# VinAIResearch/Point-Unet

Hardware: AMD Instinct MI355X
Metric: points_per_sec_forward (higher is better)
Workload: dtype f32

## Files before the change

### point-unet_amd/csrc/attpool.h

```cpp
#pragma once

#include "common.h"
#include "rowgemm.h"

namespace ps {

struct Att32Weights {
    const float* w1 = nullptr;
    const float* w2 = nullptr;
    const float* wb1 = nullptr;
    const float* wb2 = nullptr;
    const float* w1b = nullptr;
    const float* w2b = nullptr;
    const float* wb1b = nullptr;
    const float* wb2b = nullptr;
};
void pack_b3(const float* W, int cin, int cout, uint16_t* out);
void pack_b3_locse(const float* W1, int cout, uint16_t* out);
void pack_p32(const float* W, int cin, int cout, float* out);
void pack_p32_locse(const float* W1, int cout, float* out);

struct AttStage {
    const float* xyz = nullptr;
    const int32_t* idx = nullptr;
    const int32_t* order = nullptr;
    const float* fg = nullptr;
    const PackedLinear* lfa1 = nullptr;
    const PackedLinear* lfa2 = nullptr;
    const PackedLinear* wbot = nullptr;
    const PackedLinear* wfull = nullptr;
    int ldf = 0;
    float* agg = nullptr;
    int64_t n_total = 0, n_cloud = 0;
    int d = 0, k = 16;
    const Att32Weights* p32 = nullptr;
    const float* lane = nullptr;
};

constexpr int kLaneB1 = 0, kLaneW1 = 8, kLaneB2 = 88, kLaneW2 = 96, kLaneWfc = 160, kLaneImageFloats = 416;
void pack_lane_image(const float* W1, const float* b1, const float* W2, const float* b2, const float* wfc_scaled, float* out);

bool att_pool32_fits(const AttStage& s);
int att_pool32_stage(ps_context* c, const AttStage& s);
bool att_pool32b_fits(const AttStage& s);
int att_pool32b_stage(ps_context* c, const AttStage& s);

bool att_lane_fits(const ps_context* c, const AttStage& s);
int att_lane_stage(ps_context* c, const AttStage& s);
int att_lane_pass_points();

int att_pool_stage(ps_context* c, const AttStage& s);
int att_pool_form(const ps_context* c, const AttStage& s);
int att_pool16_stage(ps_context* c, const AttStage& s);

}
```

### point-unet_amd/csrc/attpool.hip

```cpp
#include "attpool.h"
#include "mfma_tile.h"

namespace ps {

struct AttArgs {
    const float* xyz;
    const int32_t* idx;
    const int32_t* order;
    const float* fg;
    const float* w1p; const float* b1;
    const float* w2p; const float* b2;
    const float* wbp;
    const float* wfp;
    float* agg;
    int n_total, n_cloud, ldf;
};

struct PointWalk {
    int t, end, stride;
    __device__ __forceinline__ PointWalk(int n_total, int units_per_wg, int unit_in_wg)
    {
        const int per_xcd = (n_total + 7) >> 3;
        const int xcd = blockIdx.x & 7, slot = blockIdx.x >> 3, slots = gridDim.x >> 3;
        t = xcd * per_xcd + slot * units_per_wg + unit_in_wg;
// ... 454 lines not shown
        if (smem > 48 * 1024) PS_HIP(hipFuncSetAttribute(reinterpret_cast<const void*>(kern), hipFuncAttributeMaxDynamicSharedMemorySize, (int)smem));
        const int blocks = (std::min(a.n_total, 256 * 16) + 7) & ~7;
        hipLaunchKernelGGL(kern, dim3(blocks), dim3(WAVES * 64), smem, c->stream, a);
        PS_HIP(hipGetLastError());
        return PS_OK;
    }
    constexpr int WAVES = per_wave * 4 <= 160 * 1024 ? 4 : (per_wave * 2 <= 160 * 1024 ? 2 : 1);
    static_assert(per_wave * WAVES <= 160 * 1024, "attention tile does not fit the LDS");
    const size_t smem = per_wave * WAVES;
    auto kern = att_kernel<D, STAGE, KN, WAVES, false>;
    if (smem > 48 * 1024) PS_HIP(hipFuncSetAttribute(reinterpret_cast<const void*>(kern), hipFuncAttributeMaxDynamicSharedMemorySize, (int)smem));
    const int blocks = (std::min(ceil_div(a.n_total, WAVES), 256 * 8) + 7) & ~7;
    hipLaunchKernelGGL(kern, dim3(blocks), dim3(WAVES * 64), smem, c->stream, a);
    PS_HIP(hipGetLastError());
    return PS_OK;
}

template <int STAGE, int KN>
static int dispatch_d(ps_context* c, int d, const AttArgs& a)
{
    switch (d) {
        case 16: return launch_att<16, STAGE, KN>(c, a);
        case 32: return launch_att<32, STAGE, KN>(c, a);
        case 64: return launch_att<64, STAGE, KN>(c, a);
        case 128: return launch_att<128, STAGE, KN>(c, a);
        case 256: return launch_att<256, STAGE, KN>(c, a);
        case 512: return launch_att<512, STAGE, KN>(c, a);
        default: set_error("att_pool: d_out %d is not a compiled size (16,32,64,128,256,512)", d); return PS_EINVAL;
    }
}

int att_pool_stage(ps_context* c, const AttStage& s)
{
    if (c->att_bf16x3 && att_pool32b_fits(s)) return att_pool32b_stage(c, s);
    if (att_pool32_fits(s)) return att_pool32_stage(c, s);
    if (att_lane_fits(c, s)) return att_lane_stage(c, s);
    return att_pool16_stage(c, s);
}

int att_pool_form(const ps_context* c, const AttStage& s)
{
    if (c->att_bf16x3 && att_pool32b_fits(s)) return 1;
    if (att_pool32_fits(s)) return 2;
    return att_lane_fits(c, s) ? 4 : 3;
}

int att_pool16_stage(ps_context* c, const AttStage& s)
{
    AttArgs a;
    a.xyz = s.xyz; a.idx = s.idx; a.order = s.order; a.fg = s.fg;
    a.w1p = s.lfa1->wp; a.b1 = s.lfa1->bias;
    a.w2p = s.lfa2 ? s.lfa2->wp : nullptr; a.b2 = s.lfa2 ? s.lfa2->bias : nullptr;
    a.wbp = s.wbot ? s.wbot->wp : nullptr;
    a.wfp = s.wfull ? s.wfull->wp : nullptr;
    a.agg = s.agg;
    a.n_total = (int)s.n_total; a.n_cloud = (int)s.n_cloud;
    a.ldf = s.ldf;
    if (s.n_total <= 0) return PS_OK;
    const int stage = s.lfa2 ? 2 : 1;
    if (s.wfull) {
        PS_CHECK((uint64_t)s.n_total * (uint64_t)std::max(s.d, std::max(s.ldf, 3 * 1)) < (1ull << 32) && (uint64_t)s.n_total * s.k < (1ull << 32),
                 "att_pool: level too large for 32-bit element offsets");
        if (s.k == 16) return stage == 1 ? dispatch_direct<1, 16>(c, s.d, a) : dispatch_direct<2, 16>(c, s.d, a);
        if (s.k == 32) return stage == 1 ? dispatch_direct<1, 32>(c, s.d, a) : dispatch_direct<2, 32>(c, s.d, a);
        set_error("att_pool: k_n %d is not a compiled size (16, 32)", s.k);
        return PS_EINVAL;
// ... 9 lines not shown
```

### point-unet_amd/csrc/attpool_lane.hip

```cpp
#include "attpool.h"
#include "mfma_tile.h"

namespace ps {

void pack_lane_image(const float* W1, const float* b1, const float* W2, const float* b2, const float* wfc_scaled, float* out)
{
    std::memcpy(out + kLaneB1, b1, sizeof(float) * 8);
    std::memcpy(out + kLaneW1, W1, sizeof(float) * 80);
    if (b2) std::memcpy(out + kLaneB2, b2, sizeof(float) * 8);
    else std::memset(out + kLaneB2, 0, sizeof(float) * 8);
    if (W2) std::memcpy(out + kLaneW2, W2, sizeof(float) * 64);
    else std::memset(out + kLaneW2, 0, sizeof(float) * 64);
    std::memcpy(out + kLaneWfc, wfc_scaled, sizeof(float) * 256);
}

namespace {

struct AttLaneArgs {
    const float* xyz;
    const int32_t* idx;
    const int32_t* order;
    const float* f;
    const float* w;
    float* agg;
    int n_total, n_cloud, ldf;
};

constexpr int kLaneWaves = 4;
constexpr int kLanePts = 4;
constexpr int kLaneMaxBlocks = 256 * 8;
constexpr int kLanePitch = 17;

static_assert(kLaneB1 == 0 && kLaneW1 == 8 && kLaneB2 == 88 && kLaneW2 == 96 && kLaneWfc == 160 && kLaneImageFloats == 13 * 32, "att_lane_kernel: image layout");

using cfloat = const float __attribute__((address_space(4)));
using cfloat2 = const f32x2 __attribute__((address_space(4)));

__device__ __forceinline__ f32x2 fma2(float x, f32x2 w, f32x2 acc) { return __builtin_elementwise_fma(f32x2{x, x}, w, acc); }
__device__ __forceinline__ f32x2 leaky2(f32x2 v) { return f32x2{leaky02(v.x), leaky02(v.y)}; }

template <int STAGE>
__global__ __launch_bounds__(kLaneWaves * 64) void att_lane_kernel(AttLaneArgs a)
{
    __shared__ float smem[kLaneWaves * 64 * kLanePitch];
    const int wave = __builtin_amdgcn_readfirstlane(threadIdx.x >> 6), lane = threadIdx.x & 63;
    const int pi = lane >> 4, k = lane & 15;
    float* T = smem + wave * (64 * kLanePitch);
    float* t_row = T + lane * kLanePitch;
    const float* t_col = T + (pi * 16) * kLanePitch + k;
    cfloat* wimg = (cfloat*)(uintptr_t)a.w;

    const bool one_cloud = a.n_total == a.n_cloud;
    const int per_xcd = ((((a.n_total + 7) >> 3) + kLanePts - 1) / kLanePts) * kLanePts;
    const int w_end = min(a.n_total, (int)((blockIdx.x & 7) + 1) * per_xcd), w_slots = gridDim.x >> 3;
    for (int t = (int)(blockIdx.x & 7) * per_xcd + ((int)(blockIdx.x >> 3) * kLaneWaves + wave) * kLanePts; t < w_end; t += w_slots * kLaneWaves * kLanePts) {
        const int ti = min(t + pi, w_end - 1);
        unsigned p, base;
        if (one_cloud) {
            p = a.order ? (unsigned)a.order[ti] : (unsigned)ti;
            base = 0u;
        } else {
            base = ((unsigned)ti / (unsigned)a.n_cloud) * (unsigned)a.n_cloud;
            p = a.order ? base + (unsigned)a.order[ti] : (unsigned)ti;
        }
        const float* cp = a.xyz + 3u * p;
        const float cx = cp[0], cy = cp[1], cz = cp[2];
        const unsigned nb = base + (unsigned)a.idx[p * 16u + (unsigned)k];
        const float* np = a.xyz + 3u * nb;
        const float nx = np[0], ny = np[1], nz = np[2];
        const float4* fr = reinterpret_cast<const float4*>(a.f + nb * (unsigned)a.ldf);
        const float4 fa = fr[0], fb = fr[1];
        const float rx = cx - nx, ry = cy - ny, rz = cz - nz;
        const float dis = __builtin_amdgcn_sqrtf(rx * rx + ry * ry + rz * rz);
        const float enc[10] = {dis, rx, ry, rz, cx, cy, cz, nx, ny, nz};

        f32x2 w[2][16];
        auto fetch = [&](int c, f32x2 (&dst)[16], auto& after) {
            cfloat* wp = wimg;
            asm volatile("" : "+s"(wp), "+v"(after));
            cfloat2* w2 = reinterpret_cast<cfloat2*>(wp) + c * 16;
#pragma unroll
            for (int j = 0; j < 16; ++j) dst[j] = w2[j];
        };
        auto mac4 = [](float xv, const f32x2* wr, f32x2 (&acc)[4]) {
#pragma unroll
            for (int j = 0; j < 4; ++j) acc[j] = fma2(xv, wr[j], acc[j]);
        };
        int tie = ti;
        fetch(0, w[0], tie);
        fetch(1, w[1], tie);
        f32x2 fx[4], g2[4];
#pragma unroll
        for (int j = 0; j < 4; ++j) fx[j] = w[0][j];
#pragma unroll
        for (int q = 0; q < 3; ++q) mac4(enc[q], &w[0][4 + 4 * q], fx);
        fetch(2, w[0], fx[0]);
#pragma unroll
        for (int q = 3; q < 7; ++q) mac4(enc[q], &w[1][4 * (q - 3)], fx);
        fetch(STAGE == 2 ? 3 : 5, w[1], fx[0]);
#pragma unroll
        for (int q = 7; q < 10; ++q) mac4(enc[q], &w[0][4 * (q - 7)], fx);
#pragma unroll
        for (int j = 0; j < 4; ++j) {
            g2[j] = w[0][12 + j];
            fx[j] = leaky2(fx[j]);
        }
        if constexpr (STAGE == 2) {
            fetch(4, w[0], g2[0]);
#pragma unroll
            for (int q = 0; q < 4; ++q) mac4(q & 1 ? fx[q >> 1].y : fx[q >> 1].x, &w[1][4 * q], g2);
            fetch(5, w[1], g2[0]);
#pragma unroll
            for (int q = 4; q < 8; ++q) mac4(q & 1 ? fx[q >> 1].y : fx[q >> 1].x, &w[0][4 * (q - 4)], g2);
#pragma unroll
            for (int j = 0; j < 4; ++j) fx[j] = leaky2(g2[j]);
        }
        const float x[16] = {fa.x, fa.y, fa.z, fa.w, fb.x, fb.y, fb.z, fb.w, fx[0].x, fx[0].y, fx[1].x, fx[1].y, fx[2].x, fx[2].y, fx[3].x, fx[3].y};
        f32x2 s[8];
#pragma unroll
        for (int j = 0; j < 8; ++j) s[j] = f32x2{0.f, 0.f};
#pragma unroll
        for (int i = 0; i < 8; ++i) {
            if (i < 7) fetch(6 + i, w[i & 1], s[0]);
            const f32x2* wr = w[(i + 1) & 1];
#pragma unroll
            for (int j = 0; j < 8; ++j) s[j] = fma2(x[2 * i], wr[j], s[j]);
#pragma unroll
            for (int j = 0; j < 8; ++j) s[j] = fma2(x[2 * i + 1], wr[8 + j], s[j]);
        }
#pragma unroll
        for (int j = 0; j < 8; ++j) {
            t_row[2 * j] = s[j].x;
            t_row[2 * j + 1] = s[j].y;
        }
        wave_lds_sync();
        float sc[16];
#pragma unroll
        for (int r = 0; r < 16; ++r) sc[r] = t_col[r * kLanePitch];
        wave_lds_sync();
#pragma unroll
        for (int q = 0; q < 16; ++q) t_row[q] = x[q];
        wave_lds_sync();
        float v[16];
#pragma unroll
        for (int r = 0; r < 16; ++r) v[r] = t_col[r * kLanePitch];
        wave_lds_sync();
        float m = sc[0];
#pragma unroll
        for (int r = 1; r < 16; ++r) m = fmaxf(m, sc[r]);
        float ss[4], num[4];
#pragma unroll
        for (int g = 0; g < 4; ++g) {
            ss[g] = 0.f;
            num[g] = 0.f;
#pragma unroll
            for (int r = 4 * g; r < 4 * g + 4; ++r) {
                const float e = __builtin_amdgcn_exp2f(sc[r] - m);
                ss[g] += e;
                num[g] = __builtin_fmaf(e, v[r], num[g]);
            }
        }
        const float ssum = (ss[0] + ss[1]) + (ss[2] + ss[3]);
        const float nsum = (num[0] + num[1]) + (num[2] + num[3]);
        if (t + pi < w_end) a.agg[p * 16u + (unsigned)k] = nsum * __builtin_amdgcn_rcpf(ssum);
    }
}

}

int att_lane_pass_points() { return kLaneMaxBlocks * kLaneWaves * kLanePts; }

bool att_lane_fits(const ps_context* c, const AttStage& s)
{
    return c->att_lane && s.wfull && s.lane && s.d == 16 && s.k == 16 && s.ldf >= 8 && s.ldf % 4 == 0 &&
           (uint64_t)s.n_total * (uint64_t)std::max(s.d, std::max(s.ldf, 3)) < (1ull << 32);
}

int att_lane_stage(ps_context* c, const AttStage& s)
{
    if (!(s.wfull && s.lane && s.d == 16 && s.k == 16)) {
        set_error("att_pool(lane): d_out %d, k_n %d -- the lane kernel is compiled for d_out 16, k_n 16 and the direct formulation only", s.d, s.k);
        return PS_EINVAL;
    }
    PS_CHECK((uint64_t)s.n_total * (uint64_t)std::max(s.d, std::max(s.ldf, 3)) < (1ull << 32), "att_pool(lane): level too large for 32-bit element offsets");
    PS_CHECK(s.ldf % 4 == 0 && s.ldf >= 8, "att_pool(lane): feature rows need a stride of whole float4s");
    if (s.n_total <= 0) return PS_OK;
    AttLaneArgs a;
    a.xyz = s.xyz; a.idx = s.idx; a.order = s.order; a.f = s.fg; a.w = s.lane; a.agg = s.agg;
    a.n_total = (int)s.n_total; a.n_cloud = (int)s.n_cloud; a.ldf = s.ldf;
    const int blocks = (std::min(ceil_div(a.n_total, kLaneWaves * kLanePts), kLaneMaxBlocks) + 7) & ~7;
    if (s.lfa2) hipLaunchKernelGGL(att_lane_kernel<2>, dim3(blocks), dim3(kLaneWaves * 64), 0, c->stream, a);
    else hipLaunchKernelGGL(att_lane_kernel<1>, dim3(blocks), dim3(kLaneWaves * 64), 0, c->stream, a);
    PS_HIP(hipGetLastError());
    return PS_OK;
}

}
```

### point-unet_amd/csrc/common.h

```cpp
#pragma once

#include <hip/hip_runtime.h>

#include <cstdarg>
#include <cstdint>
#include <cstdio>
#include <cstring>
#include <map>
#include <string>
#include <vector>

#include "../../include/pointseg.h"
#include "../../include/pointseg_train_ops.h"

namespace ps {

void set_error(const char* fmt, ...);

#define PS_HIP(expr)                                                                                  \
    do {                                                                                              \
        hipError_t _e = (expr);                                                                       \
        if (_e != hipSuccess) {                                                                       \
            ps::set_error("%s failed: %s (%s:%d)", #expr, hipGetErrorString(_e), __FILE__, __LINE__); \
            return PS_EHIP;                                                                           \
// ... 92 lines not shown
    bool gather_reduce_ordered = true;
    int maxpool_bwd_ordered = 1;
    bool train_act_bf16 = true;
    int train_att_gemm_split = -1;
    bool train_att_gemm = true;
    bool train_att128_fwd_gemm = true;
    bool train_fuse_residual = true;
    bool train_merge_syncbn = true;
    int convbn_max_c = 64;
    int convbn_rect_max = 1 << 30;
    bool wgrad_debug = false;
};
void tuning_from_env(Tuning& t);
}

struct ps_context {
    int device = 0;
    ps::Tuning tune;
    hipStream_t own_stream = nullptr;
    hipStream_t stream = nullptr;
    ps::Arena knn_arena;
    ps::Arena net_arena;
    ps::Arena sample_arena;
    ps::DevBuf stage_in;
    ps::DevBuf stage_out;
    ps::DevBuf red_ws;
    ps::DevBuf wgrad_ws;
    ps::PackCache* pack_cache = nullptr;
    ps::DevBuf ops_ring[4];
    int ops_ring_pos = 0;
    bool att_bf16x3 = true;
    bool regchain_b3 = true;
    bool att_lane = true;
    bool train_b3 = true;
    bool conv_w_transposed = false;
    bool att_df_accum = false;
    const int32_t* walk_order = nullptr;
    int64_t walk_order_n = 0;
    bool pool_bwd_overwrite = false;
    bool train_bf16 = false;
    bool train_act_bf16 = false;
    bool mid_lds_attr = false;
    size_t chain_lds_attr = 48 * 1024;
    std::map<const void*, size_t> regchain_lds_attr;
    bool deferred = false;
    int32_t* h_flags = nullptr;
    unsigned pending_mask = 0;
    uint64_t builds = 0;
    uint64_t samples = 0;
    uint64_t volume_samples = 0;
    uint64_t flag_serial[8] = {};
    int flag_kind[8] = {};
    int flag_slot = 0;
    int sticky_rc = 0;
    std::string sticky_msg;
    hipEvent_t flag_ev[8] = {};
    std::vector<char> host_ring[8];
    int ring_pos = 0;
    std::vector<char>& ring_next() { ring_pos = (ring_pos + 1) & 7; return host_ring[ring_pos]; }
    int check_deferred();
    int check_flag_slot(int s);
    int defer_status(const void* d_words, size_t bytes, int kind, uint64_t serial);
    struct PinSlot { void* p = nullptr; size_t cap = 0; hipEvent_t ev = nullptr; bool busy = false; };
    PinSlot pin[16];
    int pin_pos = 0;
    int upload_async(void* dst, const void* src, size_t bytes);
// ... 69 lines not shown
```

### point-unet_amd/csrc/debug_hooks.h

```cpp
#ifndef POINTSEG_DEBUG_H
#define POINTSEG_DEBUG_H
#include "../../include/pointseg.h"
#ifdef __cplusplus
extern "C" {
#endif
int ps_debug_knn_host(const float* support, const float* queries, int64_t B, int64_t n_support,
                      int64_t n_queries, int64_t K, int32_t* out_idx);
int ps_debug_kdtree_host(const float* support, int64_t n, int32_t* vind, int32_t* nodes, float* pts,
                         int32_t* root_depth, float* bbox);
int ps_debug_kdtree_device(ps_context* ctx, const float* support, int64_t n, int32_t* vind, int32_t* nodes,
                           float* pts, int32_t* root_depth, float* bbox);
#define PS_DEBUG_KDTREE_STATS 22
int ps_debug_kdtree_device_set(ps_context* ctx, const float* support, const int32_t* n, int64_t T, const int32_t* want_copy, int32_t* vind,
                               int32_t* nodes, float* pts, int32_t* fat, int32_t* root_depth, float* bbox, float* copy, int32_t* stats);
int ps_debug_pack_weights(const float* W, int cin, int cout, int ntb, float* out);
int ps_debug_pack_b3(const float* W, int cin, int cout, uint16_t* out);
int ps_debug_pack_b3_device(ps_context* ctx, const float* W, int cin, int cout, void* out);
int ps_debug_gemm32(ps_context* ctx, int split_bf16, const float* x1, int ld1, int c1, const int32_t* g1, const float* x2, int ld2, int c2,
                    const int32_t* g2, int gm, int gn, const float* W, const float* bias, int64_t R, int cout, int leaky, float* y, int ldy);
int ps_debug_gemm32_plan(ps_context* ctx, int split_bf16, int64_t R, int cin, int cout, int* out4);

typedef struct ps_debug_chain_layer {
    const float* W;
    const float* bias;
    int cin, cout, leaky;
    float* y;
    int ldy;
    const float* extra;
    int ld_extra, c_extra;
    const int32_t* extra_gather;
} ps_debug_chain_layer;
typedef struct ps_debug_chain_desc {
    int n_layers;
    ps_debug_chain_layer layer[4];
    const float* x1; const int32_t* g1; int ld1, c1, g1m, g1n;
    const float* x2; const int32_t* g2; int ld2, c2, g2m, g2n;
    int64_t R;
} ps_debug_chain_desc;
int ps_debug_chain(ps_context* ctx, const ps_debug_chain_desc* d, int form);
int ps_debug_chain_plan(const ps_debug_chain_desc* d, int* out4);
int ps_debug_set_regchain_b3(ps_context* ctx, int on);
int ps_debug_set_att_lane(ps_context* ctx, int on);
int ps_debug_att_stage(ps_randla* net, int level, int stage, int form, const float* xyz, const int32_t* idx, const int32_t* order, const float* fg,
                       int64_t n_total, int64_t n_cloud, float* agg);
int ps_debug_att_form(ps_randla* net, int level, int stage, int k, int64_t n_total);
int ps_debug_att_lane_pass_points(void);

int ps_debug_set_tuning(ps_context* ctx, const char* field, double value);
int ps_debug_get_tuning(ps_context* ctx, const char* field, double* value);
int ps_debug_tuning_fields(char* buf, int cap);
int ps_debug_volume_sample_args_size(void);

int64_t ps_debug_scan_words(int64_t n);
int64_t ps_debug_sort_words(int64_t n);
int ps_debug_scan_launches(int64_t n);
int ps_debug_sort_launches(int64_t n, int bits);
int ps_debug_scan_u32(ps_context* ctx, const uint32_t* in, uint32_t* out, int64_t n, uint32_t* work);
int ps_debug_sort_pairs(ps_context* ctx, int key_bytes, void* k0, void* k1, uint32_t* v0, uint32_t* v1, int64_t n, int bits, uint32_t* work,
                        int* which_out);
int ps_debug_reduce_partials(ps_context* ctx, int form, const void* part, int n_part, int nv, int n0, void* out0, void* out1);

#ifdef __cplusplus
}
#endif
#endif
```

### point-unet_amd/csrc/debug_hooks.hip

```cpp
#include "common.h"

#include <cstring>
#include <vector>
#include "kdtree_build.h"
#include "kdtree_host.h"
#include "rowgemm.h"
#include "attpool.h"
#include "debug_hooks.h"
#include "randla_net.h"
#include "reduce_partials.h"
#include "sortscan.h"

using namespace ps;

extern "C" int ps_debug_volume_sample_args_size(void) { return (int)sizeof(ps_volume_sample_args); }

extern "C" int ps_debug_pack_weights(const float* W, int cin, int cout, int ntb, float* out)
{
    PS_CHECK(W && out && (ntb == 1 || ntb == 2 || ntb == 4), "ps_debug_pack_weights: bad argument");
    pack_weights(W, cin, cout, ntb, out);
    return PS_OK;
}

extern "C" int ps_debug_pack_b3(const float* W, int cin, int cout, uint16_t* out)
// ... 243 lines not shown
    s.lane = stage == 1 ? e.lane1 : e.lane2;
    int rc = PS_EINVAL;
    if (form == 4) rc = att_lane_stage(c, s);
    else if (form == 0) rc = att_pool_stage(c, s);
    else if (form == 1 && att_pool32b_fits(s)) rc = att_pool32b_stage(c, s);
    else if (form == 2 && att_pool32_fits(s)) rc = att_pool32_stage(c, s);
    else if (form == 3) rc = att_pool16_stage(c, s);
    else set_error("ps_debug_att_stage: the level (d = %d, %lld rows) does not fit the 32x32 form %d", d, (long long)n_total, form);
    (void)hipStreamSynchronize(c->stream);
    return rc;
}

extern "C" int ps_debug_att_form(ps_randla* net, int level, int stage, int k, int64_t n_total)
{
    if (!net || !net->have_weights || level < 0 || level >= net->cfg.num_layers || (stage != 1 && stage != 2) || k < 1 || n_total < 0) {
        set_error("ps_debug_att_form: bad argument");
        return -1;
    }
    const EncLevel& e = net->enc[level];
    const int d = e.d, h = d / 2;
    const bool use_g = d >= 64;
    AttStage s;
    s.lfa1 = &e.lfa1; s.lfa2 = stage == 2 ? &e.lfa2 : nullptr;
    s.wbot = use_g ? (stage == 1 ? &e.bot1 : &e.bot2) : nullptr;
    s.wfull = use_g ? nullptr : (stage == 1 ? &e.full1 : &e.full2);
    s.lane = stage == 1 ? e.lane1 : e.lane2;
    s.p32 = e.has_p32 ? &e.p32 : nullptr;
    s.n_total = n_total; s.n_cloud = n_total; s.d = d; s.k = k; s.ldf = use_g ? h + d : h;
    return att_pool_form(net->ctx, s);
}

extern "C" int ps_debug_att_lane_pass_points(void) { return att_lane_pass_points(); }

static bool is_bool(double v) { return v == 0 || v == 1; }
static bool is_int_in(double v, double lo, double hi) { return v >= lo && v <= hi && v == (double)(int64_t)v; }

#define PS_TUNING_FIELDS(X)                                                \
    X(gemm32b_min_flops, v >= 0 && v <= 1e300)                             \
    X(gemm32b_rw, v == 0 || v == 1 || v == 2)                              \
    X(gemm32b_cw, v == 0 || v == 1 || v == 2)                              \
    X(gemm32_no_sk8, is_bool(v))                                           \
    X(att64_gemm, is_bool(v))                                              \
    X(att64_occ, v == 0 || v == 1 || v == 2)                               \
    X(att_no_split, is_bool(v))                                            \
    X(wgrad_b3_min_rows, is_int_in(v, 0, (double)(1ll << 40)))             \
    X(gemm_b3_min_rows, is_int_in(v, 0, (double)(1ll << 40)))              \
    X(wgrad_wgs, is_int_in(v, 64, 4096))                                   \
    X(bn_slice, is_bool(v))                                                \
    X(inv_bucket, is_bool(v))                                              \
    X(inv_tile, v == 4096 || v == 6144 || v == 8192)                       \
    X(gather_reduce_ordered, is_bool(v))                                   \
    X(maxpool_bwd_ordered, is_bool(v))                                     \
    X(train_act_bf16, is_bool(v))                                          \
    X(train_att_gemm_split, v == -1 || v == 0 || v == 1)                   \
    X(train_att_gemm, is_bool(v))                                          \
    X(train_att128_fwd_gemm, is_bool(v))                                   \
    X(train_fuse_residual, is_bool(v))                                     \
    X(train_merge_syncbn, is_bool(v))                                      \
    X(convbn_max_c, is_int_in(v, 0, 4096))                                 \
    X(convbn_rect_max, is_int_in(v, 0, (double)(1 << 30)))                 \
    X(wgrad_debug, is_bool(v))

extern "C" int ps_debug_set_tuning(ps_context* c, const char* field, double v)
{
    PS_CHECK(c && field, "ps_debug_set_tuning: NULL argument");
#define PS_SET(f, ok)                                                                                 \
// ... 207 lines not shown
```

### point-unet_amd/csrc/randla.hip

```cpp
#include "attpool.h"
#include "common.h"
#include "randla_net.h"
#include "rowgemm.h"

#include <memory>

namespace ps {

template <int KN>
__global__ __launch_bounds__(256) void pool_max_kernel(const float* __restrict__ feat, const int32_t* __restrict__ idx, const int32_t* __restrict__ order,
                                                       float* __restrict__ out, int rows_out, int m_cloud, int n_cloud, int K, int c4 ,
                                                       unsigned char* __restrict__ ties )
{
    const int per_xcd = (rows_out + 7) >> 3;
    const int xcd = blockIdx.x & 7;
    const size_t lim = (size_t)min(rows_out, (xcd + 1) * per_xcd) * c4;
    for (size_t t = (size_t)xcd * per_xcd * c4 + (size_t)(blockIdx.x >> 3) * 256 + threadIdx.x; t < lim; t += (size_t)(gridDim.x >> 3) * 256) {
        const int r = (int)(t / c4), q = (int)(t - (size_t)r * c4);
        const int row = order ? (r / m_cloud) * m_cloud + order[r] : r;
        const int base = (row / m_cloud) * n_cloud;
        const int32_t* ix = idx + (size_t)row * K;
        const float4* f4 = reinterpret_cast<const float4*>(feat);
        float4 m;
        if constexpr (KN > 0) {
// ... 213 lines not shown
                for (size_t t = 0; t < count; ++t) tmp[t] = (float)((double)src[t] * 1.4426950408889634);
                return tmp.data();
            };
            pack_p32(scaled(W(si + 2) + (size_t)h * d, (size_t)h * d), h, d, emit_raw(&e.p32.wb1, (size_t)h * d));
            pack_p32(W(si + 4), h, h, emit_raw(&e.p32.w2, (size_t)h * h));
            pack_p32(scaled(W(si + 5) + (size_t)h * d, (size_t)h * d), h, d, emit_raw(&e.p32.wb2, (size_t)h * d));
            if (d == 64 || d == 128 || d == 256 || d == 512) {
                pack_b3_locse(W(si + 1), h, reinterpret_cast<uint16_t*>(emit_raw(&e.p32.w1b, (size_t)(h / 32) * 3 * 64 * 4)));
                pack_b3(scaled(W(si + 2) + (size_t)h * d, (size_t)h * d), h, d, reinterpret_cast<uint16_t*>(emit_raw(&e.p32.wb1b, (size_t)h * d * 3 / 2)));
                pack_b3(W(si + 4), h, h, reinterpret_cast<uint16_t*>(emit_raw(&e.p32.w2b, (size_t)h * h * 3 / 2)));
                pack_b3(scaled(W(si + 5) + (size_t)h * d, (size_t)h * d), h, d, reinterpret_cast<uint16_t*>(emit_raw(&e.p32.wb2b, (size_t)h * d * 3 / 2)));
            }
        }
        emit(e.mlp1, W(si), Bv(si), d_in, h, 1); ++si;
        emit(e.lfa1, W(si), Bv(si), 10, h, 1); ++si;
        emit(e.top1, W(si), nullptr, h, d, 0);
        emit(e.bot1, W(si) + (size_t)h * d, nullptr, h, d, 0);
        {
            std::vector<float> sc((size_t)d * d);
            for (size_t t = 0; t < sc.size(); ++t) sc[t] = (float)((double)W(si)[t] * 1.4426950408889634);
            emit(e.full1, sc.data(), nullptr, d, d, 0);
        }
        ++si;
        emit(e.att1mlp, W(si), Bv(si), d, h, 1); ++si;
        emit(e.lfa2, W(si), Bv(si), h, h, 1); ++si;
        emit(e.top2, W(si), nullptr, h, d, 0);
        emit(e.bot2, W(si) + (size_t)h * d, nullptr, h, d, 0);
        {
            std::vector<float> sc((size_t)d * d);
            for (size_t t = 0; t < sc.size(); ++t) sc[t] = (float)((double)W(si)[t] * 1.4426950408889634);
            emit(e.full2, sc.data(), nullptr, d, d, 0);
        }
        ++si;
        e.lane1 = e.lane2 = nullptr;
        if (d == 16) {
            auto scaled16 = [&](const float* src) {
                tmp.resize(256);
                for (size_t t = 0; t < 256; ++t) tmp[t] = (float)((double)src[t] * 1.4426950408889634);
                return tmp.data();
            };
            const size_t lfa1_i = si - 5, fc1_i = si - 4, lfa2_i = si - 2, fc2_i = si - 1;
            pack_lane_image(W(lfa1_i), Bv(lfa1_i), nullptr, nullptr, scaled16(W(fc1_i)), emit_raw(&e.lane1, kLaneImageFloats));
            pack_lane_image(W(lfa1_i), Bv(lfa1_i), W(lfa2_i), Bv(lfa2_i), scaled16(W(fc2_i)), emit_raw(&e.lane2, kLaneImageFloats));
        }
        emit(e.att2mlp, W(si), Bv(si), d, d, 1); ++si;
        tmp.assign((size_t)(d + d_in) * 2 * d + 2 * d, 0.f);
        std::memcpy(tmp.data(), W(si), sizeof(float) * (size_t)d * 2 * d);
        std::memcpy(tmp.data() + (size_t)d * 2 * d, W(si + 1), sizeof(float) * (size_t)d_in * 2 * d);
        float* bsum = tmp.data() + (size_t)(d + d_in) * 2 * d;
        for (int k = 0; k < 2 * d; ++k) bsum[k] = Bv(si)[k] + Bv(si + 1)[k];
        emit(e.mlp2sc, tmp.data(), bsum, d + d_in, 2 * d, 1);
        si += 2;
        d_in = 2 * d;
    }
    emit(net->decoder0, W(si), Bv(si), d_in, d_in, 1); ++si;
    net->dec.assign(cfg.num_layers, PackedLinear());
    for (int j = 0; j < cfg.num_layers; ++j) {
        emit(net->dec[j], W(si), Bv(si), net->specs[si].cin, net->specs[si].cout, 1);
        ++si;
    }
    emit(net->fc1, W(si), Bv(si), net->specs[si].cin, 64, 1); ++si;
    emit(net->fc2, W(si), Bv(si), 64, 32, 1); ++si;
    emit(net->fc, W(si), Bv(si), 32, cfg.num_classes, 0); ++si;

    PS_TRY(net->wbuf.reserve(host.size() * sizeof(float)));
    PS_HIP(hipMemcpyAsync(net->wbuf.p, host.data(), host.size() * sizeof(float), hipMemcpyHostToDevice, c->stream));
    PS_HIP(hipStreamSynchronize(c->stream));
    for (auto& p : pend) {
        p.L->wp = net->wbuf.as<float>() + p.wp_off;
        p.L->bias = net->wbuf.as<float>() + p.b_off;
        p.L->wq = p.wq_off ? net->wbuf.as<float>() + p.wq_off : nullptr;
        p.L->w32 = p.w32_off ? net->wbuf.as<float>() + p.w32_off : nullptr;
        p.L->w32b = p.w32b_off ? net->wbuf.as<float>() + p.w32b_off : nullptr;
    }
    for (auto& p : pend_raw) *p.dst = net->wbuf.as<float>() + p.off;
    net->have_weights = true;
    return PS_OK;
}

extern "C" int ps_randla_forward(ps_randla* net, const ps_pyramid* pyr, const float* features, float* logits)
{
    PS_CHECK(net && pyr && features && logits, "ps_randla_forward: NULL argument");
    if (!net->have_weights) {
        set_error("ps_randla_forward: weights not set");
// ... 66 lines not shown
    int d_in = 8;
    for (int i = 0; i < L; ++i) {
        const EncLevel& e = net->enc[i];
        const int d = e.d, h = d / 2;
        const int64_t R = B * n[i];
        const bool use_g = d >= 64;
        const int ldf = use_g ? h + d : h;
        char nm[48];
        AttStage s;
        s.xyz = pyr->xyz[i]; s.idx = pyr->neigh_idx[i]; s.order = pyr->order[i]; s.fg = fg; s.lfa1 = &e.lfa1; s.agg = agg;
        s.n_total = R; s.n_cloud = n[i]; s.d = d; s.k = cfg.k_n; s.ldf = ldf;
        s.p32 = e.has_p32 ? &e.p32 : nullptr;
        s.lane = e.lane1;
        auto feature_rows = [&](const PackedLinear& mlp, const PackedLinear& top, const RowSrc& in) -> int {
            ChainStep ch[2] = {step(mlp, fg, ldf), step(top, fg + h, ldf)};
            const int nsteps = use_g ? 2 : 1;
            if (nsteps == 2 && rowchain_fits(ch, 2, in, none)) return rowchain(c, ch, 2, in, none, R, &net->chains);
            if (nsteps == 1 && regchain_fits(ch, 1, in, none)) return rowchain(c, ch, 1, in, none, R, &net->chains);
            PS_TRY(rowgemm(c, mlp, in, none, R, fg, ldf));
            if (use_g) PS_TRY(rowgemm(c, top, src(fg, ldf, h), none, R, fg + h, ldf));
            return PS_OK;
        };
        if (i == 0 && mlp1_0_done) {
            if (use_g) {
                std::snprintf(nm, sizeof nm, "enc%d_dense", i);
                Stage st(c, nm, 1);
                PS_TRY(rowgemm(c, e.top1, src(fg, ldf, h), none, R, fg + h, ldf));
            }
        } else {
            std::snprintf(nm, sizeof nm, "enc%d_dense", i);
            Stage st(c, nm, 1);
            PS_TRY(feature_rows(e.mlp1, e.top1, src(X, d_in, d_in)));
        }
        {
            std::snprintf(nm, sizeof nm, "enc%d_att1", i);
            Stage st(c, nm, 1);
            s.lfa2 = nullptr; s.wbot = use_g ? &e.bot1 : nullptr; s.wfull = use_g ? nullptr : &e.full1;
            PS_TRY(att_pool_stage(c, s));
        }
        {
            std::snprintf(nm, sizeof nm, "enc%d_dense", i);
            Stage st(c, nm, 1);
            PS_TRY(feature_rows(e.att1mlp, e.top2, src(agg, d, d)));
        }
        {
            std::snprintf(nm, sizeof nm, "enc%d_att2", i);
            Stage st(c, nm, 1);
            s.lfa2 = &e.lfa2; s.wbot = use_g ? &e.bot2 : nullptr; s.wfull = use_g ? nullptr : &e.full2;
            s.lane = e.lane2;
            PS_TRY(att_pool_stage(c, s));
        }
        {
            std::snprintf(nm, sizeof nm, "enc%d_dense", i);
            Stage st(c, nm, 1);
            ChainStep ch[2] = {step(e.att2mlp, nullptr, 0), step(e.mlp2sc, encb[i], 2 * d)};
            ch[1].extra = src(X, d_in, d_in);
            const RowSrc in = src(agg, d, d);
            if (rowchain_fits(ch, 2, in, none)) {
                PS_TRY(rowchain(c, ch, 2, in, none, R, &net->chains));
            } else {
                PS_TRY(rowgemm(c, e.att2mlp, in, none, R, tmp, d));
                PS_TRY(rowgemm(c, e.mlp2sc, src(tmp, d, d), src(X, d_in, d_in), R, encb[i], 2 * d));
            }
        }
        {
            std::snprintf(nm, sizeof nm, "enc%d_pool", i);
            Stage st(c, nm, 1);
            PS_TRY(pool_max(c, encb[i], pyr->sub_idx[i], i + 1 < L ? pyr->order[i + 1] : nullptr, poolb[i], B, n[i], n[i + 1], cfg.k_n, 2 * d));
        }
        tap(10 + i, encb[i], R * 2 * d);
        tap(20 + i, poolb[i], B * n[i + 1] * 2 * d);
        X = poolb[i];
        d_in = 2 * d;
    }

    {
        Stage st(c, "decoder_0", 1);
        PS_TRY(rowgemm(c, net->decoder0, src(X, d_in, d_in), none, B * n[L], dec0, d_in));
    }
    tap(30, dec0, B * n[L] * d_in);

    const float* up = dec0;
    int up_c = d_in;
    for (int j = 0; j < L; ++j) {
        const int lvl = L - 1 - j;
// ... 55 lines not shown
```

### point-unet_amd/csrc/randla_net.h

```cpp
#pragma once

#include <vector>

#include "attpool.h"
#include "common.h"
#include "rowgemm.h"

namespace ps {

struct LayerSpec {
    int cin, cout, leaky;
    size_t w_off, b_off;
};

struct EncLevel {
    PackedLinear mlp1, top1, lfa1, bot1, full1, att1mlp, lfa2, top2, bot2, full2, att2mlp, mlp2sc;
    Att32Weights p32;
    bool has_p32 = false;
    const float *lane1 = nullptr, *lane2 = nullptr;
    int d_in, d;
};

}

struct ps_randla {
    ps_context* ctx = nullptr;
    ps_randla_config cfg;
    std::vector<ps::LayerSpec> specs;
    int64_t blob_floats = 0;
    bool have_weights = false;
    ps::DevBuf wbuf;
    ps::ChainCache chains;
    ps::PackedLinear fc0, decoder0, fc1, fc2, fc;
    std::vector<ps::EncLevel> enc;
    std::vector<ps::PackedLinear> dec;
    struct Tap { int which; const float* p; int64_t count; };
    std::vector<Tap> taps;
    bool keep_taps = false;
};
```

Before: 201.8 million.

## Fuse level-0 attention MLP and shortcut layers into lane attention-pool kernel epilogue

Adds an epilogue to the lane attentive-pooling kernel for encoder level 0 (d=16, d_in=8). Stage 1 now computes the att1 MLP in-kernel and writes its 8-channel rows straight to the buffer stage 2 gathers from. Stage 2 computes the att2 MLP plus the shortcut layer and writes the 32-channel encoder output, skipping the agg round trip and two separate dense launches. The cost is extra LDS for the weight image, extra registers and wave syncs in the attention kernel, which may lower occupancy.

```diff
diff --git a/point-unet_amd/csrc/attpool.h b/point-unet_amd/csrc/attpool.h
--- a/point-unet_amd/csrc/attpool.h
+++ b/point-unet_amd/csrc/attpool.h
@@ -20,6 +20,13 @@
 void pack_p32(const float* W, int cin, int cout, float* out);
 void pack_p32_locse(const float* W1, int cout, float* out);
 
+struct AttEpilogue {
+    const float* image = nullptr;
+    float* out = nullptr;
+    int ldo = 0;
+    const float* fc0 = nullptr;
+};
+
 struct AttStage {
     const float* xyz = nullptr;
     const int32_t* idx = nullptr;
@@ -35,10 +42,15 @@
     int d = 0, k = 16;
     const Att32Weights* p32 = nullptr;
     const float* lane = nullptr;
+    const AttEpilogue* epi = nullptr;
 };
 
 constexpr int kLaneB1 = 0, kLaneW1 = 8, kLaneB2 = 88, kLaneW2 = 96, kLaneWfc = 160, kLaneImageFloats = 416;
 void pack_lane_image(const float* W1, const float* b1, const float* W2, const float* b2, const float* wfc_scaled, float* out);
+constexpr int kLaneEpi1Floats = 16 + 256, kLaneEpi2Floats = 16 + 256 + 32 + 768;
+constexpr int kLaneEpiB2 = 16 + 256, kLaneEpiW2 = kLaneEpiB2 + 32;
+void pack_lane_epilogue1(const float* W, const float* b, float* out);
+void pack_lane_epilogue2(const float* W1, const float* b1, const float* W2, const float* bsum, float* out);
 
 bool att_pool32_fits(const AttStage& s);
 int att_pool32_stage(ps_context* c, const AttStage& s);
diff --git a/point-unet_amd/csrc/attpool.hip b/point-unet_amd/csrc/attpool.hip
--- a/point-unet_amd/csrc/attpool.hip
+++ b/point-unet_amd/csrc/attpool.hip
@@ -510,6 +510,10 @@
 
 int att_pool_stage(ps_context* c, const AttStage& s)
 {
+    if (s.epi) {
+        PS_CHECK(att_lane_fits(c, s), "att_pool: only the lane kernel (d_out 16, k_n 16, the context's att_lane on) runs an epilogue");
+        return att_lane_stage(c, s);
+    }
     if (c->att_bf16x3 && att_pool32b_fits(s)) return att_pool32b_stage(c, s);
     if (att_pool32_fits(s)) return att_pool32_stage(c, s);
     if (att_lane_fits(c, s)) return att_lane_stage(c, s);
diff --git a/point-unet_amd/csrc/attpool_lane.hip b/point-unet_amd/csrc/attpool_lane.hip
--- a/point-unet_amd/csrc/attpool_lane.hip
+++ b/point-unet_amd/csrc/attpool_lane.hip
@@ -12,6 +12,26 @@
     if (W2) std::memcpy(out + kLaneW2, W2, sizeof(float) * 64);
     else std::memset(out + kLaneW2, 0, sizeof(float) * 64);
     std::memcpy(out + kLaneWfc, wfc_scaled, sizeof(float) * 256);
+}
+
+static int epi_slot_channel(int s) { return s < 16 ? 4 * (s & 3) + (s >> 2) : 16 + 4 * ((s - 16) & 1) + ((s - 16) >> 1); }
+
+static void pack_epi_layer1(const float* W, const float* b, int cout, float* out)
+{
+    for (int j = 0; j < 16; ++j) out[j] = j < cout ? b[j] : 0.f;
+    for (int s = 0; s < 16; ++s)
+        for (int j = 0; j < 16; ++j) out[16 + ((s >> 2) * 16 + j) * 4 + (s & 3)] = j < cout ? W[epi_slot_channel(s) * cout + j] : 0.f;
+}
+
+void pack_lane_epilogue1(const float* W, const float* b, float* out) { pack_epi_layer1(W, b, 8, out); }
+
+void pack_lane_epilogue2(const float* W1, const float* b1, const float* W2, const float* bsum, float* out)
+{
+    pack_epi_layer1(W1, b1, 16, out);
+    std::memcpy(out + kLaneEpiB2, bsum, sizeof(float) * 32);
+    for (int s = 0; s < 24; ++s)
+        for (int j = 0; j < 16; ++j)
+            for (int c = 0; c < 2; ++c) out[kLaneEpiW2 + ((s >> 1) * 16 + j) * 4 + (s & 1) * 2 + c] = W2[epi_slot_channel(s) * 32 + 2 * j + c];
 }
 
 namespace {
@@ -25,6 +45,11 @@
     float* agg;
     int n_total, n_cloud, ldf;
 };
+struct AttLaneEpi {
+    const float* image;
+    float* out;
+    const float* fc0;
+};
 
 constexpr int kLaneWaves = 4;
 constexpr int kLanePts = 4;
@@ -39,16 +64,28 @@
 __device__ __forceinline__ f32x2 fma2(float x, f32x2 w, f32x2 acc) { return __builtin_elementwise_fma(f32x2{x, x}, w, acc); }
 __device__ __forceinline__ f32x2 leaky2(f32x2 v) { return f32x2{leaky02(v.x), leaky02(v.y)}; }
 
-template <int STAGE>
-__global__ __launch_bounds__(kLaneWaves * 64) void att_lane_kernel(AttLaneArgs a)
-{
-    __shared__ float smem[kLaneWaves * 64 * kLanePitch];
+template <int STAGE, bool EPI = false>
+__global__ __launch_bounds__(kLaneWaves * 64) void att_lane_kernel(AttLaneArgs a, AttLaneEpi ep)
+{
+    __shared__ __attribute__((aligned(16))) float smem[kLaneWaves * 64 * kLanePitch];
+    constexpr int kEpiFloats = !EPI ? 4 : STAGE == 1 ? kLaneEpi1Floats : kLaneEpi2Floats;
+    __shared__ __attribute__((aligned(16))) float eimg[kEpiFloats];
+    if constexpr (EPI) {
+        for (int i = threadIdx.x; i < kEpiFloats / 4; i += kLaneWaves * 64) reinterpret_cast<float4*>(eimg)[i] = reinterpret_cast<const float4*>(ep.image)[i];
+        __syncthreads();
+    }
     const int wave = __builtin_amdgcn_readfirstlane(threadIdx.x >> 6), lane = threadIdx.x & 63;
     const int pi = lane >> 4, k = lane & 15;
     float* T = smem + wave * (64 * kLanePitch);
     float* t_row = T + lane * kLanePitch;
     const float* t_col = T + (pi * 16) * kLanePitch + k;
     cfloat* wimg = (cfloat*)(uintptr_t)a.w;
+    float* e_out = ep.out;
+    const float* e_fc0 = ep.fc0;
+    constexpr unsigned e_ldo = STAGE == 2 ? 32u : 8u;
+    if constexpr (EPI) {
+        asm volatile("" : "+v"(e_out), "+v"(e_fc0));
+    }
 
     const bool one_cloud = a.n_total == a.n_cloud;
     const int per_xcd = ((((a.n_total + 7) >> 3) + kLanePts - 1) / kLanePts) * kLanePts;
@@ -82,6 +119,11 @@
 #pragma unroll
             for (int j = 0; j < 16; ++j) dst[j] = w2[j];
         };
+        auto settle = [](auto& arr) {
+            if constexpr (EPI && STAGE == 2) {
+                for (auto& v : arr) asm volatile("" : "+v"(v));
+            }
+        };
         auto mac4 = [](float xv, const f32x2* wr, f32x2 (&acc)[4]) {
 #pragma unroll
             for (int j = 0; j < 4; ++j) acc[j] = fma2(xv, wr[j], acc[j]);
@@ -121,7 +163,10 @@
         for (int j = 0; j < 8; ++j) s[j] = f32x2{0.f, 0.f};
 #pragma unroll
         for (int i = 0; i < 8; ++i) {
-            if (i < 7) fetch(6 + i, w[i & 1], s[0]);
+            if (i < 7) {
+                settle(s);
+                fetch(6 + i, w[i & 1], s[0]);
+            }
             const f32x2* wr = w[(i + 1) & 1];
 #pragma unroll
             for (int j = 0; j < 8; ++j) s[j] = fma2(x[2 * i], wr[j], s[j]);
@@ -162,7 +207,77 @@
         }
         const float ssum = (ss[0] + ss[1]) + (ss[2] + ss[3]);
         const float nsum = (num[0] + num[1]) + (num[2] + num[3]);
-        if (t + pi < w_end) a.agg[p * 16u + (unsigned)k] = nsum * __builtin_amdgcn_rcpf(ssum);
+        float pooled = nsum * __builtin_amdgcn_rcpf(ssum);
+        if constexpr (!EPI) {
+            if (t + pi < w_end) a.agg[p * 16u + (unsigned)k] = pooled;
+        } else {
+            auto layer16 = [&](const float* at, const float* wl, float bias) {
+                float in[16];
+#pragma unroll
+                for (int g = 0; g < 4; ++g) {
+                    const float4 r = reinterpret_cast<const float4*>(at)[g];
+                    in[4 * g] = r.x; in[4 * g + 1] = r.y; in[4 * g + 2] = r.z; in[4 * g + 3] = r.w;
+                }
+                float acc = 0.f;
+#pragma unroll
+                for (int q = 0; q < 4; ++q) {
+                    const float4 wv = reinterpret_cast<const float4*>(wl)[q * 16];
+                    acc = __builtin_fmaf(in[q], wv.x, acc);
+                    acc = __builtin_fmaf(in[4 + q], wv.y, acc);
+                    acc = __builtin_fmaf(in[8 + q], wv.z, acc);
+                    acc = __builtin_fmaf(in[12 + q], wv.w, acc);
+                }
+                return leaky02(acc + bias);
+            };
+            unsigned tid = threadIdx.x;
+            asm volatile("" : "+v"(tid));
+            const unsigned ek = tid & 15u;
+            float* Te = smem + (tid >> 6) * (64 * kLanePitch);
+            float* te_lane = Te + (tid & 63u);
+            const float* te_pt = Te + (tid & 48u);
+            const float* ew = eimg + 4u * ek;
+            float4 sa = {}, sb = {};
+            if constexpr (STAGE == 2) {
+                const float4* xr = reinterpret_cast<const float4*>(e_fc0 + p * 8u);
+                asm volatile("" : "+v"(xr), "+v"(pooled));
+                sa = xr[0];
+                sb = xr[1];
+            }
+            te_lane[0] = pooled;
+            wave_lds_sync();
+            const float f1 = layer16(te_pt, ew + 16, eimg[ek]);
+            if constexpr (STAGE == 1) {
+                if (ek < 8 && t + pi < w_end) e_out[p * e_ldo + ek] = f1;
+            } else {
+                te_lane[64] = f1;
+                wave_lds_sync();
+                float in[24];
+#pragma unroll
+                for (int g = 0; g < 4; ++g) {
+                    const float4 r = reinterpret_cast<const float4*>(te_pt + 64)[g];
+                    in[4 * g] = r.x; in[4 * g + 1] = r.y; in[4 * g + 2] = r.z; in[4 * g + 3] = r.w;
+                }
+                in[16] = sa.x; in[17] = sa.y; in[18] = sa.z; in[19] = sa.w;
+                in[20] = sb.x; in[21] = sb.y; in[22] = sb.z; in[23] = sb.w;
+                f32x2 acc = f32x2{0.f, 0.f};
+                const float4* w2 = reinterpret_cast<const float4*>(ew + kLaneEpiW2);
+#pragma unroll
+                for (int s2 = 0; s2 < 12; ++s2) {
+                    if (s2 % 3 == 0 && s2 > 0) asm volatile("" : "+v"(w2), "+v"(acc));
+                    const float4 wv = w2[s2 * 16];
+#pragma unroll
+                    for (int e = 0; e < 2; ++e) {
+                        const int s = 2 * s2 + e;
+                        const int ch = s < 16 ? 4 * (s & 3) + (s >> 2) : 16 + 4 * ((s - 16) & 1) + ((s - 16) >> 1);
+                        acc = fma2(in[ch], e ? f32x2{wv.z, wv.w} : f32x2{wv.x, wv.y}, acc);
+                    }
+                }
+                const f32x2 bs = *reinterpret_cast<const f32x2*>(eimg + kLaneEpiB2 + 2 * ek);
+                const f32x2 y = leaky2(acc + bs);
+                if (t + pi < w_end) *reinterpret_cast<f32x2*>(e_out + p * e_ldo + 2u * ek) = y;
+            }
+            wave_lds_sync();
+        }
     }
 }
 
@@ -173,7 +288,8 @@
 bool att_lane_fits(const ps_context* c, const AttStage& s)
 {
     return c->att_lane && s.wfull && s.lane && s.d == 16 && s.k == 16 && s.ldf >= 8 && s.ldf % 4 == 0 &&
-           (uint64_t)s.n_total * (uint64_t)std::max(s.d, std::max(s.ldf, 3)) < (1ull << 32);
+           (uint64_t)s.n_total * (uint64_t)std::max(s.d, std::max(s.ldf, 3)) < (1ull << 32) &&
+           (!s.epi || (uint64_t)s.n_total * (uint64_t)s.epi->ldo < (1ull << 32));
 }
 
 int att_lane_stage(ps_context* c, const AttStage& s)
@@ -188,9 +304,24 @@
     AttLaneArgs a;
     a.xyz = s.xyz; a.idx = s.idx; a.order = s.order; a.f = s.fg; a.w = s.lane; a.agg = s.agg;
     a.n_total = (int)s.n_total; a.n_cloud = (int)s.n_cloud; a.ldf = s.ldf;
+    AttLaneEpi ep = {nullptr, nullptr, nullptr};
+    const int stage = s.lfa2 ? 2 : 1;
+    if (s.epi) {
+        const AttEpilogue& e = *s.epi;
+        const int cout = stage == 2 ? 32 : 8;
+        PS_CHECK(e.image && e.out && (stage == 1 || e.fc0), "att_pool(lane): the stage-%d epilogue needs its image, its output rows%s", stage, stage == 2 ? " and the shortcut rows" : "");
+        PS_CHECK(e.ldo == cout, "att_pool(lane): the stage-%d epilogue is compiled for dense output rows of %d floats, not a stride of %d", stage, cout, e.ldo);
+        PS_CHECK((uint64_t)s.n_total * (uint64_t)e.ldo < (1ull << 32), "att_pool(lane): level too large for 32-bit element offsets");
+        PS_CHECK((const void*)e.out != (const void*)s.fg, "att_pool(lane): the epilogue cannot store into the rows the stage gathers from");
+        PS_CHECK(reinterpret_cast<uintptr_t>(e.image) % 16 == 0 && reinterpret_cast<uintptr_t>(e.out) % 8 == 0 && reinterpret_cast<uintptr_t>(e.fc0) % 16 == 0,
+                 "att_pool(lane): epilogue image, output and shortcut rows must be 16 / 8 / 16-byte aligned");
+        ep.image = e.image; ep.out = e.out; ep.fc0 = e.fc0;
+    }
     const int blocks = (std::min(ceil_div(a.n_total, kLaneWaves * kLanePts), kLaneMaxBlocks) + 7) & ~7;
-    if (s.lfa2) hipLaunchKernelGGL(att_lane_kernel<2>, dim3(blocks), dim3(kLaneWaves * 64), 0, c->stream, a);
-    else hipLaunchKernelGGL(att_lane_kernel<1>, dim3(blocks), dim3(kLaneWaves * 64), 0, c->stream, a);
+    if (s.epi && stage == 2) hipLaunchKernelGGL((att_lane_kernel<2, true>), dim3(blocks), dim3(kLaneWaves * 64), 0, c->stream, a, ep);
+    else if (s.epi) hipLaunchKernelGGL((att_lane_kernel<1, true>), dim3(blocks), dim3(kLaneWaves * 64), 0, c->stream, a, ep);
+    else if (s.lfa2) hipLaunchKernelGGL(att_lane_kernel<2>, dim3(blocks), dim3(kLaneWaves * 64), 0, c->stream, a, ep);
+    else hipLaunchKernelGGL(att_lane_kernel<1>, dim3(blocks), dim3(kLaneWaves * 64), 0, c->stream, a, ep);
     PS_HIP(hipGetLastError());
     return PS_OK;
 }
diff --git a/point-unet_amd/csrc/common.h b/point-unet_amd/csrc/common.h
--- a/point-unet_amd/csrc/common.h
+++ b/point-unet_amd/csrc/common.h
@@ -148,6 +148,7 @@
     bool att_bf16x3 = true;
     bool regchain_b3 = true;
     bool att_lane = true;
+    unsigned att_lane_epi = 3;
     bool train_b3 = true;
     bool conv_w_transposed = false;
     bool att_df_accum = false;
diff --git a/point-unet_amd/csrc/debug_hooks.h b/point-unet_amd/csrc/debug_hooks.h
--- a/point-unet_amd/csrc/debug_hooks.h
+++ b/point-unet_amd/csrc/debug_hooks.h
@@ -45,6 +45,10 @@
                        int64_t n_total, int64_t n_cloud, float* agg);
 int ps_debug_att_form(ps_randla* net, int level, int stage, int k, int64_t n_total);
 int ps_debug_att_lane_pass_points(void);
+int ps_debug_set_att_lane_epilogue(ps_context* ctx, int stages);
+int ps_debug_att_epilogue_routed(ps_randla* net, int level, int stage, int k, int64_t n_total);
+int ps_debug_att_lane_epilogue(ps_randla* net, int stage, int epilogue, const float* xyz, const int32_t* idx, const int32_t* order, const float* f,
+                               const float* fc0, int64_t n_total, int64_t n_cloud, float* agg, float* out);
 
 int ps_debug_set_tuning(ps_context* ctx, const char* field, double value);
 int ps_debug_get_tuning(ps_context* ctx, const char* field, double* value);
diff --git a/point-unet_amd/csrc/debug_hooks.hip b/point-unet_amd/csrc/debug_hooks.hip
--- a/point-unet_amd/csrc/debug_hooks.hip
+++ b/point-unet_amd/csrc/debug_hooks.hip
@@ -299,6 +299,72 @@
 
 extern "C" int ps_debug_att_lane_pass_points(void) { return att_lane_pass_points(); }
 
+extern "C" int ps_debug_set_att_lane_epilogue(ps_context* c, int stages)
+{
+    PS_CHECK(c && stages >= 0 && stages <= 3, "ps_debug_set_att_lane_epilogue: bad argument");
+    c->att_lane_epi = (unsigned)stages;
+    return PS_OK;
+}
+
+extern "C" int ps_debug_att_epilogue_routed(ps_randla* net, int level, int stage, int k, int64_t n_total)
+{
+    if (!net || !net->have_weights || level < 0 || level >= net->cfg.num_layers || (stage != 1 && stage != 2) || k < 1 || n_total < 0) {
+        set_error("ps_debug_att_epilogue_routed: bad argument");
+        return -1;
+    }
+    const EncLevel& e = net->enc[level];
+    const int d = e.d, h = d / 2;
+    const bool use_g = d >= 64;
+    AttStage s;
+    s.lfa1 = &e.lfa1; s.lfa2 = stage == 2 ? &e.lfa2 : nullptr;
+    s.wbot = use_g ? (stage == 1 ? &e.bot1 : &e.bot2) : nullptr;
+    s.wfull = use_g ? nullptr : (stage == 1 ? &e.full1 : &e.full2);
+    s.lane = stage == 1 ? e.lane1 : e.lane2;
+    s.p32 = e.has_p32 ? &e.p32 : nullptr;
+    s.n_total = n_total; s.n_cloud = n_total; s.d = d; s.k = k; s.ldf = use_g ? h + d : h;
+    return lane_epilogue_routed(net->ctx, e, level, stage, s) ? 1 : 0;
+}
+
+extern "C" int ps_debug_att_lane_epilogue(ps_randla* net, int stage, int epilogue, const float* xyz, const int32_t* idx, const int32_t* order, const float* f,
+                                          const float* fc0, int64_t n_total, int64_t n_cloud, float* agg, float* out)
+{
+    PS_CHECK(net && xyz && idx && f && agg && out && (stage == 1 || fc0), "ps_debug_att_lane_epilogue: NULL argument");
+    PS_CHECK(net->have_weights, "ps_debug_att_lane_epilogue: weights not set");
+    PS_CHECK((stage == 1 || stage == 2) && (epilogue == 0 || epilogue == 1), "ps_debug_att_lane_epilogue: bad stage / epilogue");
+    PS_CHECK(n_total >= 0 && n_cloud >= 1 && n_total % n_cloud == 0, "ps_debug_att_lane_epilogue: n_total must be a whole number of clouds");
+    ps_context* c = net->ctx;
+    PS_HIP(hipSetDevice(c->device));
+    const EncLevel& e = net->enc[0];
+    PS_CHECK(e.epi1 && e.epi2, "ps_debug_att_lane_epilogue: level 0 of this network (d_out %d) has no epilogue images", e.d);
+    const int d = e.d, h = d / 2;
+    AttStage s;
+    s.xyz = xyz; s.idx = idx; s.order = order; s.fg = f; s.lfa1 = &e.lfa1; s.agg = agg;
+    s.n_total = n_total; s.n_cloud = n_cloud; s.d = d; s.k = net->cfg.k_n; s.ldf = h;
+    s.lfa2 = stage == 2 ? &e.lfa2 : nullptr;
+    s.wfull = stage == 1 ? &e.full1 : &e.full2;
+    s.lane = stage == 1 ? e.lane1 : e.lane2;
+    AttEpilogue ep;
+    ep.image = stage == 1 ? e.epi1 : e.epi2; ep.out = out; ep.ldo = stage == 1 ? h : 2 * d; ep.fc0 = stage == 2 ? fc0 : nullptr;
+    if (epilogue) s.epi = &ep;
+    int rc = att_lane_stage(c, s);
+    if (rc == PS_OK && !epilogue && n_total > 0) {
+        RowSrc in, none;
+        in.x = agg; in.ld = d; in.c = d;
+        ChainStep ch[2];
+        if (stage == 1) {
+            ch[0].L = &e.att1mlp; ch[0].y = out; ch[0].ldy = h;
+            rc = rowchain(c, ch, 1, in, none, n_total, &net->chains);
+        } else {
+            ch[0].L = &e.att2mlp;
+            ch[1].L = &e.mlp2sc; ch[1].y = out; ch[1].ldy = 2 * d;
+            ch[1].extra.x = fc0; ch[1].extra.ld = e.d_in; ch[1].extra.c = e.d_in;
+            rc = rowchain(c, ch, 2, in, none, n_total, &net->chains);
+        }
+    }
+    (void)hipStreamSynchronize(c->stream);
+    return rc;
+}
+
 static bool is_bool(double v) { return v == 0 || v == 1; }
 static bool is_int_in(double v, double lo, double hi) { return v >= lo && v <= hi && v == (double)(int64_t)v; }
 
diff --git a/point-unet_amd/csrc/randla.hip b/point-unet_amd/csrc/randla.hip
--- a/point-unet_amd/csrc/randla.hip
+++ b/point-unet_amd/csrc/randla.hip
@@ -269,7 +269,7 @@
             emit(e.full2, sc.data(), nullptr, d, d, 0);
         }
         ++si;
-        e.lane1 = e.lane2 = nullptr;
+        e.lane1 = e.lane2 = e.epi1 = e.epi2 = nullptr;
         if (d == 16) {
             auto scaled16 = [&](const float* src) {
                 tmp.resize(256);
@@ -287,6 +287,11 @@
         float* bsum = tmp.data() + (size_t)(d + d_in) * 2 * d;
         for (int k = 0; k < 2 * d; ++k) bsum[k] = Bv(si)[k] + Bv(si + 1)[k];
         emit(e.mlp2sc, tmp.data(), bsum, d + d_in, 2 * d, 1);
+        if (d == 16 && d_in == 8) {
+            const size_t att1mlp_i = si - 4, att2mlp_i = si - 1;
+            pack_lane_epilogue1(W(att1mlp_i), Bv(att1mlp_i), emit_raw(&e.epi1, kLaneEpi1Floats));
+            pack_lane_epilogue2(W(att2mlp_i), Bv(att2mlp_i), tmp.data(), bsum, emit_raw(&e.epi2, kLaneEpi2Floats));
+        }
         si += 2;
         d_in = 2 * d;
     }
@@ -419,13 +424,21 @@
             Stage st(c, nm, 1);
             PS_TRY(feature_rows(e.mlp1, e.top1, src(X, d_in, d_in)));
         }
+        AttEpilogue ep1, ep2;
         {
             std::snprintf(nm, sizeof nm, "enc%d_att1", i);
             Stage st(c, nm, 1);
             s.lfa2 = nullptr; s.wbot = use_g ? &e.bot1 : nullptr; s.wfull = use_g ? nullptr : &e.full1;
+            if (lane_epilogue_routed(c, e, i, 1, s)) {
+                ep1.image = e.epi1; ep1.out = tmp; ep1.ldo = h;
+                s.epi = &ep1;
+            }
             PS_TRY(att_pool_stage(c, s));
         }
-        {
+        if (s.epi) {
+            s.epi = nullptr;
+            s.fg = tmp;
+        } else {
             std::snprintf(nm, sizeof nm, "enc%d_dense", i);
             Stage st(c, nm, 1);
             PS_TRY(feature_rows(e.att1mlp, e.top2, src(agg, d, d)));
@@ -435,9 +448,13 @@
             Stage st(c, nm, 1);
             s.lfa2 = &e.lfa2; s.wbot = use_g ? &e.bot2 : nullptr; s.wfull = use_g ? nullptr : &e.full2;
             s.lane = e.lane2;
+            if (lane_epilogue_routed(c, e, i, 2, s)) {
+                ep2.image = e.epi2; ep2.out = encb[i]; ep2.ldo = 2 * d; ep2.fc0 = X;
+                s.epi = &ep2;
+            }
             PS_TRY(att_pool_stage(c, s));
         }
-        {
+        if (!s.epi) {
             std::snprintf(nm, sizeof nm, "enc%d_dense", i);
             Stage st(c, nm, 1);
             ChainStep ch[2] = {step(e.att2mlp, nullptr, 0), step(e.mlp2sc, encb[i], 2 * d)};
diff --git a/point-unet_amd/csrc/randla_net.h b/point-unet_amd/csrc/randla_net.h
--- a/point-unet_amd/csrc/randla_net.h
+++ b/point-unet_amd/csrc/randla_net.h
@@ -18,8 +18,14 @@
     Att32Weights p32;
     bool has_p32 = false;
     const float *lane1 = nullptr, *lane2 = nullptr;
+    const float *epi1 = nullptr, *epi2 = nullptr;
     int d_in, d;
 };
+
+inline bool lane_epilogue_routed(const ps_context* c, const EncLevel& e, int level, int stage, const AttStage& s)
+{
+    return level == 0 && (c->att_lane_epi >> (stage - 1) & 1u) && (stage == 1 ? e.epi1 : e.epi2) && e.d_in == 8 && !s.epi && att_lane_fits(c, s);
+}
 
 }
 
```

New measurement: 202.8 million, median of 6. Within noise of the previous version (+0.5%).
